# CHEBSB/PolarDecoding

Hardware: AMD Instinct MI355X
Metric: decoded frames/sec, N=1024 K=512 CA-SCL L=8 (higher is better)
Workload: dtype f64

## Files before the change

### polardecoding_amd/csrc/scl_fast2.h

```cpp
#pragma once
#include "fast2_lds.h"
#include "fast2_scratch.h"
#include "octet_bits.h"
#include "scl_fast.h"

namespace polar {

template <typename R>
struct Fast2Cfg {
    static constexpr int NLOG = 10, N = 1024, NW = 32, TOP = 9, HI = 8, L = 8;
    static constexpr int NA = 32;
    static constexpr int WAVES = 4;
    static constexpr int MIN_WAVES_PER_SIMD = sizeof(R) == 8 ? 3 : 4;
    static constexpr int NFA = HI - 3;
    static constexpr size_t sc_l8 = fast2_scratch::SC_L8;
    static constexpr size_t sc_l7 = fast2_scratch::SC_L7;
    static constexpr size_t sc_l6 = fast2_scratch::SC_L6;
    static constexpr size_t sc_tl = fast2_scratch::SC_TL;
    static constexpr size_t scratch_cw = fast2_scratch::SCRATCH_CW;
    static constexpr size_t scratch_elems = 2 * scratch_cw;
    static constexpr bool PAIRED = sizeof(R) == 8;
    static constexpr bool TOP_WORDS_ONCE = sizeof(R) == 8;
    static constexpr size_t off_lut = 0;
    static constexpr size_t off_frz = off_lut + ((Lut<R>::bytes + 15) / 16) * 16;
    static constexpr size_t off_msk = off_frz + 4 * NW;
    static constexpr size_t off_kth = off_msk + 4 * CRC_MASK_ROWS * NW;
    static constexpr size_t off_stair = off_kth + 256 * 8;
    static constexpr size_t shared_bytes = off_stair + ((Stair<R>::bytes + 15) / 16) * 16;
    static constexpr size_t off_bl = 0;
    static constexpr size_t off_cw = off_bl + 4 * fast2_lds::ROWS_WORDS;
    static constexpr size_t off_cd = off_cw + 4 * fast2_lds::ROWS_WORDS;
    static constexpr size_t off_ky = off_cd + sizeof(R) * 32;
    static constexpr size_t off_sg = off_ky + 128;
    static constexpr size_t per_wave = off_sg + sizeof(R) * 512;
    static constexpr size_t total = shared_bytes + WAVES * per_wave;
    static_assert(off_cw % 16 == 0 && off_cd % 16 == 0 && per_wave % 16 == 0 && shared_bytes % 16 == 0, "LDS regions are 16-byte aligned");
};
static_assert(3 * Fast2Cfg<double>::total <= 163840 && 4 * Fast2Cfg<float>::total <= 163840, "the pair kernel's LDS limits its occupancy");

template <int QP>
__device__ __forceinline__ double quadp(double x) { return quad_lanes<QP>(x); }
template <int QP>
__device__ __forceinline__ float quadp(float x) { return quad_lanes<QP>(x); }

template <bool FROM_Y>
struct Fast2Sigma { double sigma; };
template <>
struct Fast2Sigma<false> {};

template <typename R, typename IN, bool CRC_ON, bool FROM_Y>
struct Fast2Dec : Fast2Sigma<FROM_Y> {
    using C = Fast2Cfg<R>;
    static constexpr int N = C::N, NW = C::NW, TOP = C::TOP, HI = C::HI, L = 8, NFA = C::NFA;

    R A[C::NA];
    R a1;
    R bp_s, bp_d, bp_ts, bp_td;
    R PM;
    uint32_t ptr, bl0, fl;
    int logact;
    int p, c, pos, lane, gl;
    int own_addr, oth_addr;
    uint32_t pos0_mask;
    int cand_addr;
    Lut<R> lut;
    R *cand, *stg;
    uint32_t *blw, *curw, *keys;
    const unsigned char *kth;
    __amdgpu_buffer_rsrc_t rs_scr;
    __amdgpu_buffer_rsrc_t rs_in;
    unsigned cscr;
    unsigned csrc;
    static __device__ __forceinline__ __amdgpu_buffer_rsrc_t make_rsrc(const void *base, unsigned bytes)
    {
        return __builtin_amdgcn_make_buffer_rsrc(const_cast<void *>(base), 0, (int)bytes, 0x00020000);
    }
    typedef unsigned u2_t __attribute__((ext_vector_type(2)));
    static __device__ __forceinline__ double ld_buf(__amdgpu_buffer_rsrc_t r, unsigned eoff, double, int aux)
    {
        return aux ? __builtin_bit_cast(double, __builtin_amdgcn_raw_buffer_load_b64(r, eoff * 8u, 0, 16))
                   : __builtin_bit_cast(double, __builtin_amdgcn_raw_buffer_load_b64(r, eoff * 8u, 0, 0));
    }
    static __device__ __forceinline__ float ld_buf(__amdgpu_buffer_rsrc_t r, unsigned eoff, float, int aux)
    {
        return aux ? __builtin_bit_cast(float, __builtin_amdgcn_raw_buffer_load_b32(r, eoff * 4u, 0, 16))
                   : __builtin_bit_cast(float, __builtin_amdgcn_raw_buffer_load_b32(r, eoff * 4u, 0, 0));
    }
    static __device__ __forceinline__ void st_buf(__amdgpu_buffer_rsrc_t r, unsigned eoff, double v)
    {
        __builtin_amdgcn_raw_buffer_store_b64(__builtin_bit_cast(u2_t, v), r, eoff * 8u, 0, 0);
    }
    static __device__ __forceinline__ void st_buf(__amdgpu_buffer_rsrc_t r, unsigned eoff, float v)
    {
        __builtin_amdgcn_raw_buffer_store_b32(__builtin_bit_cast(unsigned, v), r, eoff * 4u, 0, 0);
    }
    typedef unsigned u4_t __attribute__((ext_vector_type(4)));
    struct R2 {
        R a, b;
    };
    static __device__ __forceinline__ R2 ld_buf2(__amdgpu_buffer_rsrc_t r, unsigned eoff, int aux)
    {
        static_assert(sizeof(R2) == 16, "paired accesses are for f64");
        return aux ? __builtin_bit_cast(R2, __builtin_amdgcn_raw_buffer_load_b128(r, eoff * 8u, 0, 16))
                   : __builtin_bit_cast(R2, __builtin_amdgcn_raw_buffer_load_b128(r, eoff * 8u, 0, 0));
    }
    static __device__ __forceinline__ void st_buf2(__amdgpu_buffer_rsrc_t r, unsigned eoff, R2 v)
    {
        static_assert(sizeof(R2) == 16, "paired accesses are for f64");
        __builtin_amdgcn_raw_buffer_store_b128(__builtin_bit_cast(u4_t, v), r, eoff * 8u, 0, 0);
    }
    struct SPtr {
        const Fast2Dec *d;
        unsigned off;
        struct Ref {
            const Fast2Dec *d;
            unsigned off;
            __device__ __forceinline__ void operator=(R v) const { st_buf(d->rs_scr, off, v); }
        };
        __device__ __forceinline__ SPtr operator+(int k) const { return SPtr{d, off + (unsigned)k}; }
        __device__ __forceinline__ Ref operator[](int k) const { return Ref{d, off + (unsigned)k}; }
    };
    static __device__ __forceinline__ R ld_sc(SPtr q) { return ld_buf(q.d->rs_scr, q.off, R(0), 1); }
    static __device__ __forceinline__ int sg(int e) { return C::PAIRED ? (int)fast2_scratch::sigma((unsigned)e) : e; }
    static __device__ __forceinline__ int sg2(int pos, int m) { return C::PAIRED ? (int)fast2_scratch::pair_at((unsigned)pos, (unsigned)m) : pos + 8 * m; }
    static __device__ __forceinline__ R2 ld_sc2(SPtr q)
    {
        if constexpr (C::PAIRED) return ld_buf2(q.d->rs_scr, q.off, 1);
        else return R2{ld_sc(q), ld_sc(q + sg(4))};
    }
    static __device__ __forceinline__ void st_sc2(SPtr q, R a, R b)
    {
        if constexpr (C::PAIRED) st_buf2(q.d->rs_scr, q.off, R2{a, b});
        else {
            q[0] = a;
            q[sg(4)] = b;
        }
    }

    static __device__ __forceinline__ int row(int slot) { return fast2_lds::row(slot); }
    __device__ __forceinline__ int pa(int t) const { return (ptr >> (3 * (t - 4))) & 7; }
    __device__ __forceinline__ void set_pa(int t, int v) { ptr = (ptr & ~(7u << (3 * (t - 4)))) | ((uint32_t)v << (3 * (t - 4))); }
    __device__ __forceinline__ int pb(int t) const { return (ptr >> (3 * (NFA + t - 5))) & 7; }
    __device__ __forceinline__ void set_pb(int t, int v) { ptr = (ptr & ~(7u << (3 * (NFA + t - 5)))) | ((uint32_t)v << (3 * (NFA + t - 5))); }
    __device__ __forceinline__ R chk(R a, R b) const { return chk_lut1<R>(a, b, lut); }
    __device__ __forceinline__ R chks(R a, R b) const { return chk_lut1<R>(a, b, lut); }
    __device__ __forceinline__ R chv(int e) const
    {
        double v = (double)ld_buf(rs_in, csrc + (unsigned)e, IN(0), 0);
        if constexpr (FROM_Y) v = llr_from_y(v, this->sigma);
        return (R)v;
    }
    static __device__ __forceinline__ unsigned fresh(unsigned off)
    {
        __asm__ volatile("" : "+v"(off));
        return off;
    }
    __device__ __forceinline__ SPtr l8(int slot) const { return SPtr{this, fresh(cscr + (unsigned)(C::sc_l8 + slot * 256))}; }
    __device__ __forceinline__ SPtr l7(int slot) const { return SPtr{this, fresh(cscr + (unsigned)(C::sc_l7 + slot * 128))}; }
    __device__ __forceinline__ SPtr tls() const { return SPtr{this, fresh(cscr + (unsigned)C::sc_tl)}; }

    template <int T>
    __device__ __forceinline__ void f_reg()
    {
        constexpr int RO = (1 << T) / 4;
#pragma unroll
        for (int r = 0; r < RO; ++r) A[RO + r] = chk(A[2 * RO + r], A[3 * RO + r]);
        if constexpr (T >= 4) set_pa(T, p);
    }
    template <int T>
    __device__ __forceinline__ void g_reg()
    {
        constexpr int RO = (1 << T) / 4;
        const int sl = pa(T + 1) * 8 + gl;
        uint32_t w;
        if constexpr (T == 5) w = blw[row(pb(5)) + 1] >> pos;
        else w = bl0 >> (16 + pos);
#pragma unroll
        for (int r = 0; r < RO; ++r) {
            const R x = __shfl(A[2 * RO + r], sl), y = __shfl(A[3 * RO + r], sl);
            A[RO + r] = g_bit<R>(x, y, w, 4 * r);
        }
        set_pa(T, p);
    }
    __device__ __forceinline__ void g3()
    {
        const int sl = pa(4) * 8 + gl;
        const uint32_t w = bl0 >> (8 + pos);
#pragma unroll
        for (int r = 0; r < 2; ++r) {
            const R x = __shfl(A[4 + r], sl), y = __shfl(A[6 + r], sl);
            A[2 + r] = g_bit<R>(x, y, w, 4 * r);
        }
    }

    __device__ __forceinline__ void push_l6(R v)
    {
#pragma unroll
        for (int r = 16; r < 31; ++r) A[r] = A[r + 1];
        A[31] = v;
    }
    __device__ __forceinline__ void load_l6() { set_pa(6, p); }
    __device__ __forceinline__ R top_src(bool right, int idx, int q) const
    {
        const int seg = idx >> 4, within = idx & 15;
        const int e = 16 * q + within + 64 * (seg & 3) + 256 * (seg >> 2);
        return right ? chv(e) : ld_sc(tls() + e);
    }
    __device__ __forceinline__ void from_top(bool right, bool gstep)
    {
        vm_drain();
        const uint32_t *bt = blw + row(pb(TOP)) + 16;
        const uint32_t *bh = blw + row(pb(HI)) + 8;
        const SPtr o8 = l8(p), o7 = l7(p);
        const int w32 = (int)fresh((unsigned)(p * 4 + pos));
        const int nld = right ? 8 : 4;
        R *pre = A + 4;
#pragma unroll
        for (int m = 0; m < 8; ++m) pre[m] = (m < nld) ? top_src(right, w32 + 32 * m, 0) : R(0);
        uint32_t wt[8] = {0, 0, 0, 0, 0, 0, 0, 0}, wh[4] = {0, 0, 0, 0};
        for (int q = 0; q < 4; ++q) {
            lds_fence();
#pragma unroll
            for (int m = 0; m < 8; ++m)
                if (m < nld) stg[w32 + 32 * m] = pre[m];
            if (C::TOP_WORDS_ONCE && (q & 1) == 0) {
                const int wq = q >> 1;
#pragma unroll
                for (int k = 0; k < 4; ++k) {
                    if (right) {
                        wt[k] = bt[2 * k + wq] >> pos;
                        wt[4 + k] = bt[8 + 2 * k + wq] >> pos;
                    }
                    if (gstep) wh[k] = bh[2 * k + wq] >> pos;
                }
            }
            lds_fence();
            if (q < 3) {
#pragma unroll
                for (int m = 0; m < 8; ++m) pre[m] = (m < nld) ? top_src(right, w32 + 32 * m, q + 1) : R(0);
            }
#pragma unroll 1
            for (int i = 0; i < 4; ++i) {
                const int rr = 4 * q + i;
                const int s0 = sg(pos + 4 * rr);
                const int sh = 4 * (rr & 7);
                const int wq = rr >> 3;
                const int wi = 4 * i + pos;
                R *v8 = A + 12;
#pragma unroll
                for (int k = 0; k < 4; ++k) {
                    R x, y;
                    if (right) {
                        const uint32_t w0 = C::TOP_WORDS_ONCE ? wt[k] : bt[2 * k + wq] >> pos;
                        const uint32_t w1 = C::TOP_WORDS_ONCE ? wt[4 + k] : bt[8 + 2 * k + wq] >> pos;
                        x = g_bit<R>(stg[(k + 0) * 16 + wi], stg[(k + 8) * 16 + wi], w0, sh);
                        y = g_bit<R>(stg[(k + 4) * 16 + wi], stg[(k + 12) * 16 + wi], w1, sh);
                    } else {
                        x = stg[(k + 0) * 16 + wi];
                        y = stg[(k + 4) * 16 + wi];
                    }
                    if (gstep) v8[k] = g_bit<R>(x, y, C::TOP_WORDS_ONCE ? wh[k] : bh[2 * k + wq] >> pos, sh);
                    else v8[k] = chk(x, y);
                    o8[s0 + 64 * k] = v8[k];
                }
                const R v70 = chk(v8[0], v8[2]), v71 = chk(v8[1], v8[3]);
                o7[s0] = v70;
                o7[s0 + 64] = v71;
                push_l6(chk(v70, v71));
            }
        }
        set_pa(8, p);
        set_pa(7, p);
        load_l6();
    }
    __device__ __forceinline__ void from_l8()
    {
        vm_drain();
        const SPtr s8 = l8(pa(8));
        const uint32_t *b7 = blw + row(pb(7)) + 4;
        const SPtr o7 = l7(p);
        constexpr int CP = sizeof(R) == 8 ? 2 : 4;
        static_assert(CP % 2 == 0 && 4 * CP <= 16, "a chunk is whole pairs of passes and fits the dead registers");
        for (int q = 0; q < 16 / CP; ++q) {
            R *in = A;
#pragma unroll
            for (int j = 0; j < CP / 2; ++j) {
                const int m = CP / 2 * q + j;
#pragma unroll
                for (int k = 0; k < 4; ++k) {
                    const R2 v = ld_sc2(s8 + sg2(pos, m) + 64 * k);
                    in[8 * j + k] = v.a;
                    in[8 * j + 4 + k] = v.b;
                }
            }
#pragma unroll
            for (int j = 0; j < CP / 2; ++j) {
                const int m = CP / 2 * q + j;
                R v70[2], v71[2];
#pragma unroll
                for (int h = 0; h < 2; ++h) {
                    const int i = 2 * j + h;
                    const int rr = CP * q + i;
                    const int sh = 4 * (rr & 7);
                    const int wq = rr >> 3;
                    v70[h] = g_bit<R>(in[4 * i], in[4 * i + 2], b7[wq] >> pos, sh);
                    v71[h] = g_bit<R>(in[4 * i + 1], in[4 * i + 3], b7[2 + wq] >> pos, sh);
                }
                st_sc2(o7 + sg2(pos, m), v70[0], v70[1]);
                st_sc2(o7 + sg2(pos, m) + 64, v71[0], v71[1]);
                push_l6(chk(v70[0], v71[0]));
                push_l6(chk(v70[1], v71[1]));
            }
        }
        set_pa(7, p);
        load_l6();
    }
    __device__ __forceinline__ void from_l7()
    {
        vm_drain();
        const SPtr s7 = l7(pa(7));
        const uint32_t *b6 = blw + row(pb(6)) + 2;
        const uint32_t w0 = b6[0] >> pos, w1 = b6[1] >> pos;
#pragma unroll
        for (int m = 0; m < 8; ++m) {
            const R2 x = ld_sc2(s7 + sg2(pos, m)), y = ld_sc2(s7 + sg2(pos, m) + 64);
            const int r = 2 * m;
            A[16 + r] = g_bit<R>(x.a, y.a, r < 8 ? w0 : w1, 4 * (r & 7));
            A[17 + r] = g_bit<R>(x.b, y.b, r < 8 ? w0 : w1, 4 * ((r + 1) & 7));
        }
        set_pa(6, p);
    }

    __device__ __forceinline__ void octet_head(int o)
    {
        const int d = (o == 0) ? 10 : 3 + __builtin_ctz((unsigned)o);
        if (d >= 8) from_top(o >= N / 16, d == 8);
        else if (d == 7) from_l8();
        else if (d == 6) from_l7();
        else if (d == 5) g_reg<5>();
        else if (d == 4) g_reg<4>();
        else g3();
        if (d > 5) f_reg<5>();
        if (d > 4) f_reg<4>();
        if (d > 3) f_reg<3>();
    }
    __device__ __forceinline__ void octet_head_reg(int o)
    {
        const int d = 3 + __builtin_ctz((unsigned)o);
        if (d == 5) g_reg<5>();
        else if (d == 4) g_reg<4>();
        else g3();
        if (d > 4) f_reg<4>();
        if (d > 3) f_reg<3>();
    }

    template <int K>
    __device__ __forceinline__ void set_bit_k(int o, uint32_t bit)
    {
        if constexpr (K < 7) {
            bl0 |= bit << K;
        } else {
            const uint32_t c3 = octet_bits::level3((bl0 & 0x7Fu) | (bit << 7));
            bl0 &= ~0xFFu;
            set_bit7(o, c3);
        }
    }
    __device__ __forceinline__ void set_bit7(int o, uint32_t c3)
    {
        if ((o & 1) == 0) {
            bl0 = (bl0 & ~0xFF00u) | (c3 << 8);
            return;
        }
        const uint32_t c4 = (((bl0 >> 8) & 0xFFu) ^ c3) | (c3 << 8);
        if ((o & 2) == 0) {
            bl0 = (bl0 & 0xFFFFu) | (c4 << 16);
            return;
        }
        set_bit_lds(8 * o + 7, ((bl0 >> 16) ^ c4) | (c4 << 16));
    }
    __device__ __forceinline__ void set_bit_lds(int j, uint32_t cur)
    {
        const int own = (int)fresh((unsigned)row(p));
        lds_fence();
        if (pos == 0) curw[own] = cur;
        lds_fence();
        int t = 5;
        while (t < 10 && ((j >> t) & 1)) {
            const int nw = 1 << (t - 5);
            const int sb = pb(t);
            for (int w = pos; w < nw; w += 4) {
                const uint32_t cc = curw[own + w];
                const uint32_t l = blw[row(sb) + nw + w];
                curw[own + w] = l ^ cc;
                curw[own + w + nw] = cc;
            }
            lds_fence();
            ++t;
        }
        if (t < 10) {
            const int nw = 1 << (t - 5);
            for (int w = pos; w < nw; w += 4) blw[own + nw + w] = curw[own + w];
            set_pb(t, p);
            lds_fence();
        }
    }

    __device__ __forceinline__ uint32_t survivors(R c0, R c1)
    {
        lds_fence();
        if (pos == 0) {
            keys[2 * p] = metric_key(c0);
            keys[2 * p + 1] = metric_key(c1);
        }
        lds_fence();
        const unsigned char *kb = reinterpret_cast<const unsigned char *>(keys) - 64 * c;
        const uint32_t own = *reinterpret_cast<const uint32_t *>(kb + own_addr);
        const uint32_t oth = *reinterpret_cast<const uint32_t *>(kb + oth_addr);
        const uint32_t own1 = own + 1u;
        uint32_t acc = (oth - own1) >> 31;
        acc = __builtin_amdgcn_alignbit(acc, (uint32_t)dpp_i<0x121>((int)oth) - own1, 31);
        acc = __builtin_amdgcn_alignbit(acc, (uint32_t)dpp_i<0x122>((int)oth) - own1, 31);
        acc = __builtin_amdgcn_alignbit(acc, (uint32_t)dpp_i<0x123>((int)oth) - own1, 31);
        acc = __builtin_amdgcn_alignbit(acc, (uint32_t)dpp_i<0x124>((int)oth) - own1, 31);
        acc = __builtin_amdgcn_alignbit(acc, (uint32_t)dpp_i<0x125>((int)oth) - own1, 31);
        acc = __builtin_amdgcn_alignbit(acc, (uint32_t)dpp_i<0x126>((int)oth) - own1, 31);
        acc = __builtin_amdgcn_alignbit(acc, (uint32_t)dpp_i<0x127>((int)oth) - own1, 31);
        uint32_t cnt = __popc(acc);
        {
            auto r = __builtin_amdgcn_permlane16_swap(cnt, cnt, false, false);
            cnt = r[0] + r[1];
        }
        uint64_t b = __ballot(cnt <= (uint32_t)L);
        uint32_t m_a = (uint32_t)b & 0xFFFFu, m_b = (uint32_t)(b >> 32) & 0xFFFFu;
        if (sizeof(R) == 8 && (__popc(m_a) != L || __popc(m_b) != L)) {
            if (__popc(c ? m_b : m_a) != L) fl |= 0x4u;
            lds_fence();
            if (pos == 0) {
                cand[p] = c0;
                cand[8 + p] = c1;
            }
            lds_fence();
            const R *cb = reinterpret_cast<const R *>(reinterpret_cast<const unsigned char *>(cand) - (int)sizeof(R) * 16 * c);
            const R *mycand = reinterpret_cast<const R *>(reinterpret_cast<const unsigned char *>(cb) + cand_addr);
            const R mine = mycand[lane & 15];
            int n = 0;
#pragma unroll
            for (int m = 0; m < 16; ++m) n += (mycand[m] <= mine) ? 1 : 0;
            b = __ballot(n <= L);
            m_a = (uint32_t)b & 0xFFFFu;
            m_b = (uint32_t)(b >> 32) & 0xFFFFu;
        }
        return c ? m_b : m_a;
    }

    __device__ __forceinline__ bool trivial_prune(R cb, R cw) const
    {
        uint32_t mx = metric_key(cb) & pos0_mask;
        mx = max(mx, (uint32_t)dpp_i<0x128>((int)mx));
        {
            auto a = __builtin_amdgcn_permlane16_swap(mx, mx, false, false);
            mx = max(a[0], a[1]);
        }
        {
            auto a = __builtin_amdgcn_permlane32_swap(mx, mx, false, false);
            mx = max(a[0], a[1]);
        }
        return __ballot(mx >= (metric_key(cw) | ~pos0_mask)) == 0ull;
    }
    static __device__ __forceinline__ uint32_t sign_bit(double x) { return (uint32_t)__double2hiint(x) >> 31; }
    static __device__ __forceinline__ uint32_t sign_bit(float x) { return (uint32_t)__float_as_int(x) >> 31; }

    template <int K, bool FULL>
    __device__ __forceinline__ void decide(int o, bool frozen, R lam) { decide_t<K, FULL>(o, frozen, lam, lut.tabv(lam)); }
    template <int K, bool FULL>
    __device__ __forceinline__ void decide_t(int o, bool frozen, R lam, R tt)
    {
        if (frozen) {
            PM += tt + negmax(lam);
            set_bit_k<K>(o, 0u);
            return;
        }
        uint32_t bit;
        R pm;
        if (!FULL && logact < 3) {
            const R ph0 = tt + negmax(lam), ph1 = tt + posmax(lam);
            bit = (p >> logact) & 1;
            pm = PM + (bit ? ph1 : ph0);
            ++logact;
        } else {
            const uint32_t lneg = sign_bit(lam);
            const R cb = PM + tt, cw = PM + (tt + absr(lam));
            bit = (uint32_t)dpp_i<0x00>((int)lneg);
            pm = cb;
            if (!trivial_prune(cb, cw)) ranked<K>(lneg, cb, cw, bit, pm);
        }
        PM = pm;
        set_bit_k<K>(o, bit);
    }
    template <int K>
    __device__ __forceinline__ void ranked(uint32_t lneg, R cb, R cw, uint32_t &bit, R &pm)
    {
        const R c0 = lneg ? cw : cb, c1 = lneg ? cb : cw;
        const uint32_t mask = survivors(c0, c1);
        const uint32_t m0 = mask & 0xFFu, m1 = mask >> 8;
        const uint32_t m_both = m0 & m1, m_dead = ~(m0 | m1) & 0xFFu;
        if (__popc(mask) < L) fl |= 0x1u;
        const bool s0 = (m0 >> p) & 1, s1 = (m1 >> p) & 1;
        bit = (!s0 && s1) ? 1u : 0u;
        pm = bit ? c1 : c0;
        if (__ballot(m_dead != 0u) == 0ull) return;
        const bool dead = !s0 && !s1;
        const int myrank = __popc(m_dead & ((1u << p) - 1u));
        const bool refilled = dead && (myrank < __popc(m_both));
        const int src = (int)kth[m_both * 8 + myrank];
        const int sg = refilled ? src : p;
        const int sl = sg * 8 + gl;
        const R c1s = __shfl(c1, sl);
        ptr = __shfl(ptr, sl);
        bl0 = __shfl(bl0, sl);
        if constexpr ((K & 4) == 0) { A[2] = __shfl(A[2], sl); A[3] = __shfl(A[3], sl); }
        if constexpr ((K & 2) == 0) { A[1] = __shfl(A[1], sl); a1 = __shfl(a1, sl); }
        if constexpr ((K & 1) == 0) { bp_d = __shfl(bp_d, sl); bp_td = __shfl(bp_td, sl); }
        bit = refilled ? 1u : bit;
        pm = refilled ? c1s : pm;
    }

    __device__ __forceinline__ void frozen_prefix(int P, int nphi, bool regs, R &xl, R &yl)
    {
        const int w32 = p * 4 + pos, j0 = 8 * P;
        vm_drain();
        {
            const SPtr tl = tls();
            const SPtr o8 = l8(0) + sg(w32), o7 = l7(0) + sg(w32);
            R v8[8];
#pragma unroll
            for (int k = 0; k < 8; ++k) {
                const int e = w32 + 32 * k;
                v8[k] = chk(ld_sc(tl + e), ld_sc(tl + e + 256));
                o8[32 * k] = v8[k];
            }
            lds_fence();
#pragma unroll
            for (int k = 0; k < 4; ++k) {
                const R v7 = chk(v8[k], v8[k + 4]);
                o7[32 * k] = v7;
                stg[w32 + 32 * k] = v7;
            }
            set_pa(8, 0);
            set_pa(7, 0);
        }
        lds_fence();
#pragma unroll
        for (int t = 6; t >= 0; --t) {
            const int h = 1 << t;
            int idx[2];
            R x[2], y[2];
#pragma unroll
            for (int i = 0; i < 2; ++i) {
                const int b = w32 + 32 * i;
                idx[i] = ((b >> t) << (t + 1)) | (b & (h - 1));
                x[i] = stg[idx[i]];
                y[i] = stg[idx[i] + h];
            }
            if (t == 0) {
                xl = stg[126];
                yl = stg[127];
            }
            lds_fence();
#pragma unroll
            for (int i = 0; i < 2; ++i) {
                stg[idx[i]] = chk(x[i], y[i]);
                stg[idx[i] + h] = y[i] + x[i];
            }
            lds_fence();
            if (t >= 4 && regs) {
                const R *node = stg + ((j0 >> t) << t) + pos;
#pragma unroll
                for (int r = 0; r < h / 4; ++r) A[h / 4 + r] = node[4 * r];
            }
        }
#pragma unroll
        for (int k = 0; k < 4; ++k) {
            const R lam = stg[w32 + 32 * k];
            stg[128 + w32 + 32 * k] = lut.tabv(lam) + negmax(lam);
        }
        lds_fence();
        R pm = PM;
#pragma unroll 8
        for (int j = 0; j < nphi; ++j) pm += stg[128 + j];
        PM = pm;
        lds_fence();
    }

    __device__ __forceinline__ uint32_t fill_tail(uint32_t f2, R lam0, R xl, R yl)
    {
        uint32_t b0 = 0, b1 = 0;
        if (!(f2 & 1u)) {
            b0 = (p >> logact) & 1;
            ++logact;
        }
        PM += lut.tabv(lam0) + (b0 ? posmax(lam0) : negmax(lam0));
        const R lam1 = b0 ? -(xl - yl) : yl + xl;
        if (!(f2 & 2u)) {
            b1 = (p >> logact) & 1;
            ++logact;
        }
        PM += lut.tabv(lam1) + (b1 ? posmax(lam1) : negmax(lam1));
        return (b0 ? 0x55555555u : 0u) ^ (b1 ? 0xFFFFFFFFu : 0u);
    }
    __device__ __forceinline__ void fill_phase(int E, const uint32_t *frz, R xl, R yl)
    {
        const int w32 = (int)fresh((unsigned)(p * 4 + pos));
        const int qb = (p & 1) * 64;
        const uint32_t wv0 = fill_tail(frz[3] >> 30, stg[126], xl, yl);
        uint32_t wv1 = 0;
        lds_fence();
        blw[row(p) + 4 + pos] = wv0;
        lds_fence();
#pragma unroll 1
        for (int S = 128; S < E; S += 64) {
            vm_drain();
            const uint32_t wsel = S == 128 ? wv0 : wv1;
            uint32_t wq[2];
            wq[0] = (uint32_t)__shfl((int)wsel, gl) >> w32;
            wq[1] = (uint32_t)__shfl((int)wsel, 8 + gl) >> w32;
            if (S == 128) {
                const SPtr s8 = l8(0) + sg(w32);
                R v8[8];
#pragma unroll
                for (int k = 0; k < 8; ++k) v8[k] = ld_sc(s8 + 32 * k);
#pragma unroll
                for (int q = 0; q < 2; ++q) {
                    const SPtr o7 = l7(q) + sg(w32);
                    R v7[4];
#pragma unroll
                    for (int k = 0; k < 4; ++k) {
                        v7[k] = g_bit<R>(v8[k], v8[k + 4], wq[q], 0);
                        o7[32 * k] = v7[k];
                    }
                    stg[64 * q + w32] = chk(v7[0], v7[2]);
                    stg[64 * q + w32 + 32] = chk(v7[1], v7[3]);
                }
                set_pa(7, p & 1);
            } else {
#pragma unroll
                for (int q = 0; q < 2; ++q) {
                    const SPtr s7 = l7(q) + sg(w32);
#pragma unroll
                    for (int i = 0; i < 2; ++i)
                        stg[64 * q + w32 + 32 * i] = g_bit<R>(ld_sc(s7 + 32 * i), ld_sc(s7 + 32 * i + 64), wq[q], 0);
                }
            }
            lds_fence();
#pragma unroll
            for (int t = 5; t >= 0; --t) {
                const int h = 1 << t;
                int idx[2];
                R x[2], y[2];
#pragma unroll
                for (int i = 0; i < 2; ++i) {
                    const int b = w32 + 32 * i;
                    idx[i] = ((b >> t) << (t + 1)) | (b & (h - 1));
                    x[i] = stg[idx[i]];
                    y[i] = stg[idx[i] + h];
                }
                if (t == 0) {
                    xl = stg[qb + 62];
                    yl = stg[qb + 63];
                }
                lds_fence();
#pragma unroll
                for (int i = 0; i < 2; ++i) {
                    stg[idx[i]] = chk(x[i], y[i]);
                    stg[idx[i] + h] = y[i] + x[i];
                }
                lds_fence();
            }
#pragma unroll
            for (int k = 0; k < 4; ++k) {
                const R lam = stg[w32 + 32 * k];
                stg[128 + w32 + 32 * k] = lut.tabv(lam) + negmax(lam);
            }
            lds_fence();
            R pm = PM;
#pragma unroll 2
            for (int j = 0; j < 62; ++j) pm += stg[128 + qb + j];
            PM = pm;
            const uint32_t wv = fill_tail(frz[(S + 62) >> 5] >> 30, stg[qb + 62], xl, yl);
            lds_fence();
            if (S == 128) {
                wv1 = wv;
                if (pos < 2) blw[row(p) + 2 + pos] = wv;
            } else {
                const uint32_t b = pos < 2 ? wv1 ^ wv : wv;
                blw[row(p) + 8 + pos] = wv0 ^ b;
                blw[row(p) + 12 + pos] = b;
            }
            lds_fence();
        }
    }

    template <bool FULL>
    __device__ __forceinline__ void octet_frozen_prefix(int o, bool last_frozen)
    {
        R xf = chks(A[2], A[3]), xg = A[3] + A[2];
        R yf = quadp<0x4E>(xf), yg = quadp<0x4E>(xg);
        {
            const R ff = chks(xf, yf), gf = xf + yf, fg = chks(xg, yg), gg = xg + yg;
            xf = (pos & 2) ? gf : ff;
            xg = (pos & 2) ? gg : fg;
        }
        yf = quadp<0xB1>(xf); yg = quadp<0xB1>(xg);
        R lf, lg;
        {
            const R ff = chks(xf, yf), gf = xf + yf, fg = chks(xg, yg), gg = xg + yg;
            lf = (pos & 1) ? gf : ff;
            lg = (pos & 1) ? gg : fg;
        }
        const R pf = lut.tabv(lf) + negmax(lf), pg = lut.tabv(lg) + negmax(lg);
        PM += pf;
        PM += quadp<0x55>(pf);
        PM += quadp<0xAA>(pf);
        PM += quadp<0xFF>(pf);
        PM += pg;
        PM += quadp<0x55>(pg);
        PM += quadp<0xAA>(pg);
        if (last_frozen) {
            PM += quadp<0xFF>(pg);
            set_bit7(o, 0u);
        } else {
            decide<7, FULL>(o, false, quadp<0xFF>(lg));
        }
    }

    struct ChkBp { R v, s, d, ts, td; };
    static __device__ __forceinline__ R g_sel(R sum, R dif, uint32_t w, int sh)
    {
        const uint32_t m = (uint32_t)__builtin_amdgcn_sbfe((int)w, sh, 1);
        return Lut<R>::sel_mask(m, -dif, sum);
    }
    static __device__ __forceinline__ double flip_sign(double y, uint32_t m) { return __hiloint2double(__double2hiint(y) ^ (int)m, __double2loint(y)); }
    static __device__ __forceinline__ float flip_sign(float y, uint32_t m) { return __int_as_float(__float_as_int(y) ^ (int)m); }
    template <int QP>
    __device__ __forceinline__ ChkBp chk_narrow(R x) const
    {
        static_assert(QP == 0xB1 || QP == 0x4E, "partner in lane ^ 1 or lane ^ 2");
        const uint32_t up = QP == 0xB1 ? (uint32_t)pos << 31 : ((uint32_t)pos << 30) & 0x80000000u;
        const R y = flip_sign(quadp<QP>(x), up);
        ChkBp r;
        r.s = x + y;
        r.d = x - y;
        r.ts = lut.tabv(r.s);
        r.td = quadp<QP>(r.ts);
        r.v = xor_sign(minabs(x, y), x, y) + (r.ts - r.td);
        return r;
    }
    template <int K, bool FULL>
    __device__ __forceinline__ void leaf_pair(int o, uint32_t fm, R x1)
    {
        const ChkBp q = chk_narrow<0xB1>(x1);
        bp_d = q.d;
        bp_td = q.td;
        decide<K, FULL>(o, (fm >> K) & 1, q.v);
        const uint32_t m1 = (uint32_t)__builtin_amdgcn_sbfe((int)bl0, K, 1);
        decide_t<K + 1, FULL>(o, (fm >> (K + 1)) & 1, Lut<R>::sel_mask(m1, -bp_d, q.s), Lut<R>::sel_mask(m1, bp_td, q.ts));
    }
    template <bool FULL>
    __device__ __forceinline__ void octet(int o, uint32_t fm)
    {
        {
            const R s2 = A[2] + A[3], d2 = A[2] - A[3];
            const R v2 = xor_sign(minabs(A[2], A[3]), A[2], A[3]) + (lut.tabv(s2) - lut.tabv(d2));
            A[2] = s2;
            A[3] = d2;
            const ChkBp q1 = chk_narrow<0x4E>(v2);
            A[1] = q1.s;
            a1 = q1.d;
            leaf_pair<0, FULL>(o, fm, q1.v);
        }
        leaf_pair<2, FULL>(o, fm, g_sel(A[1], a1, octet_bits::level1_lo(bl0), pos));
        {
            const R v2 = g_sel(A[2], A[3], octet_bits::level2(bl0), pos);
            const ChkBp q1 = chk_narrow<0x4E>(v2);
            A[1] = q1.s;
            a1 = q1.d;
            leaf_pair<4, FULL>(o, fm, q1.v);
        }
        leaf_pair<6, FULL>(o, fm, g_sel(A[1], a1, octet_bits::level1_hi(bl0), pos));
    }
};

template <typename D, bool FULL>
__device__ __forceinline__ int octet_group(D &s, const uint32_t *frz, uint32_t &fword, int o)
{
    s.octet_head(o);
    for (;;) {
        if ((o & 3) == 0) fword = frz[o >> 2];
        const uint32_t fm = (fword >> (8 * (o & 3))) & 0xFFu;
        if ((fm & 0x7Fu) != 0x7Fu) s.template octet<FULL>(o, fm);
        else s.template octet_frozen_prefix<FULL>(o, fm == 0xFFu);
        ++o;
        if ((o & 7) == 0) break;
        s.octet_head_reg(o);
    }
    return o;
}

template <typename R, typename IN, bool CRC_ON, bool FROM_Y>
__device__ __forceinline__ void scl_fast2_body(const SclParams &P)
{
    using D = Fast2Dec<R, IN, CRC_ON, FROM_Y>;
    using C = Fast2Cfg<R>;
    constexpr int N = C::N, NW = C::NW, L = 8;
    extern __shared__ __attribute__((aligned(16))) unsigned char smem[];
    const int wave = __builtin_amdgcn_readfirstlane(threadIdx.x >> 6);
    unsigned char *base = smem + C::shared_bytes + (size_t)wave * C::per_wave;
    uint32_t *frz = reinterpret_cast<uint32_t *>(smem + C::off_frz);
    uint32_t *msk = reinterpret_cast<uint32_t *>(smem + C::off_msk);
    unsigned char *kth = smem + C::off_kth;

    Lut<R>::build(smem + C::off_lut, threadIdx.x, blockDim.x);
    for (int i = threadIdx.x; i < NW; i += blockDim.x) frz[i] = P.frozen[i];
    if (CRC_ON)
        for (int i = threadIdx.x; i < CRC_MASK_ROWS * NW; i += blockDim.x)
            msk[i] = P.crc_mask[(i & ~(NW - 1)) + ((i >> 3) & 3) + 4 * (i & 7)];
    for (int i = threadIdx.x; i < 256 * 8; i += blockDim.x) {
        int m = i >> 3, k = i & 7, idx = 0, seen = 0;
        for (int b = 0; b < 8; ++b)
            if ((m >> b) & 1) {
                if (seen == k) idx = b;
                ++seen;
            }
        kth[i] = (unsigned char)idx;
    }
    __syncthreads();

    D s;
    s.lane = threadIdx.x & 63;
    s.p = s.lane >> 3;
    s.c = (s.lane >> 2) & 1;
    s.pos = s.lane & 3;
    s.pos0_mask = s.pos == 0 ? 0xFFFFFFFFu : 0u;
    s.gl = s.lane & 7;
    s.lut.bind(smem + C::off_lut);
    s.kth = kth;
    s.blw = reinterpret_cast<uint32_t *>(base + C::off_bl) + fast2_lds::cw_base(1) * s.c;
    s.curw = reinterpret_cast<uint32_t *>(base + C::off_cw) + fast2_lds::cw_base(1) * s.c;
    s.cand = reinterpret_cast<R *>(base + C::off_cd) + s.c * 16;
    s.keys = reinterpret_cast<uint32_t *>(base + C::off_ky) + s.c * 16;
    s.stg = reinterpret_cast<R *>(base + C::off_sg) + s.c * 256;
    if constexpr (FROM_Y) s.sigma = P.sigma;
    {
        const int i = s.lane & 15, row = s.lane >> 4, cwr = row >> 1, h = row & 1;
        const int jj = (i + 8 * h) & 15;
        s.own_addr = 64 * cwr + 4 * (2 * (i & 7) + (i >> 3));
        s.oth_addr = 64 * cwr + 4 * (2 * (jj & 7) + (jj >> 3));
        s.cand_addr = (int)sizeof(R) * 16 * cwr;
    }
    const int lane = s.lane, p = s.p, c = s.c, pos = s.pos;
    const int wave_global = blockIdx.x * C::WAVES + wave;
    const int waves_total = gridDim.x * C::WAVES;
    R *scr_wave = reinterpret_cast<R *>(P.scratch) + (size_t)wave_global * C::scratch_elems;
    s.rs_scr = D::make_rsrc(scr_wave, (unsigned)(C::scratch_elems * sizeof(R)));
    s.cscr = (unsigned)c * (unsigned)C::scratch_cw;

    int lead = 0;
    while (lead < 15 && ((frz[lead >> 2] >> (8 * (lead & 3))) & 0xFFu) == 0xFFu) ++lead;
    lead = __builtin_amdgcn_readfirstlane(lead);
    const int E = P.fill_end;

    for (int pair = wave_global; 2 * pair < P.B;) {
        const int frame_raw = 2 * pair + c;
        const bool live = frame_raw < P.B;
        const int frame = live ? frame_raw : P.B - 1;
        s.rs_in = D::make_rsrc(reinterpret_cast<const IN *>(P.in) + (size_t)(2 * pair) * N, (unsigned)(2 * N * sizeof(IN)));
        s.csrc = (unsigned)(frame - 2 * pair) * (unsigned)N;
        {
            const auto t = s.tls();
            const int w = p * 4 + pos;
#pragma unroll 2
            for (int e = w; e < N / 2; e += 32) t[e] = s.chk(s.chv(e), s.chv(e + N / 2));
        }
#pragma unroll
        for (int j = 0; j < NW / 4; ++j) s.blw[D::row(p) + pos + 4 * j] = 0;
        lds_fence();

        s.PM = R(0);
        s.ptr = 0;
        for (int t = 4; t <= 8; ++t) s.set_pa(t, p);
        for (int t = 5; t <= 9; ++t) s.set_pb(t, p);
        s.bl0 = 0;
        s.a1 = R(0);
#pragma unroll
        for (int r = 0; r < C::NA; ++r) s.A[r] = R(0);
        s.fl = 0;
        s.logact = 0;
        uint32_t fword = 0;

        int o_first = 0;
        if (E > 0 || lead > 0) {
            R xl, yl;
            s.frozen_prefix(E > 0 ? 15 : lead, E > 0 ? 126 : 8 * lead, E == 0, xl, yl);
            o_first = lead;
            if (E > 0) {
                s.fill_phase(E, frz, xl, yl);
                o_first = E >> 3;
            }
            fword = frz[o_first >> 2];
        }
        int o = o_first;
#pragma unroll 1
        while (o < N / 8 && s.logact < 3) o = octet_group<D, false>(s, frz, fword, o);
        while (o < N / 8) o = octet_group<D, true>(s, frz, fword, o);

        bool pass = false;
        if constexpr (CRC_ON) {
            lds_fence();
            uint32_t x[8];
#pragma unroll
            for (int j = 0; j < 8; ++j) x[j] = s.curw[D::row(p) + pos + 4 * j];
            typedef uint32_t u4_t __attribute__((ext_vector_type(4)));
            const u4_t *mk = reinterpret_cast<const u4_t *>(msk + 8 * pos);
            const int rows = (P.crc_r + 3) & ~3;
            uint32_t rem = 0;
#pragma unroll 1
            for (int i = 0; i < rows; i += 4) {
#pragma unroll
                for (int k = 0; k < 4; ++k) {
                    const u4_t a = mk[(i + k) * (NW / 4)], b = mk[(i + k) * (NW / 4) + 1];
                    const uint32_t acc = (x[0] & a.x) ^ (x[1] & a.y) ^ (x[2] & a.z) ^ (x[3] & a.w) ^ (x[4] & b.x) ^
                                         (x[5] & b.y) ^ (x[6] & b.z) ^ (x[7] & b.w);
                    rem |= (uint32_t)(__popc(acc) & 1) << (i + k);
                }
            }
            rem ^= (uint32_t)dpp_i<0xB1>((int)rem);
            rem ^= (uint32_t)dpp_i<0x4E>((int)rem);
            pass = rem == 0u;
        }
        const uint64_t bp_ = __ballot(pass && pos == 0);
        const uint64_t cwmask = 0x0101010101010101ull << (4 * c);
        const bool any = (bp_ & cwmask) != 0ull;
        int best = -1;
        R best_pm = R(0);
        for (int q = 0; q < L; ++q) {
            const R pq = __shfl(s.PM, q * 8 + 4 * c);
            const int okq = __shfl((int)(any ? pass : true), q * 8 + 4 * c);
            if (okq && (best < 0 || pq < best_pm)) {
                best = q;
                best_pm = pq;
            }
        }
        uint32_t fl = s.fl;
        if (any) fl |= 0x2u;
        lds_fence();
        {
            const int w = p * 4 + pos;
            uint32_t x = s.curw[D::row(best) + w];
            x = polar_word_transform(x);
#pragma unroll
            for (int hw = 1; hw < NW; hw <<= 1) {
                const int wo = w ^ hw;
                const uint32_t ov = __shfl(x, (wo >> 2) * 8 + 4 * c + (wo & 3));
                if (!(w & hw)) x ^= ov;
            }
            if (live) P.out_bits[(size_t)frame * NW + w] = x;
        }
        if (live && p == 0 && pos == 0) {
            if (P.pm) P.pm[frame] = (double)best_pm;
            if (P.flags) P.flags[frame] = fl;
        }
        lds_fence();
        pair = next_job_wave(P.queue, pair, waves_total, (P.B + 1) >> 1);
    }
}

template <typename R, typename IN, bool CRC_ON>
__global__ __launch_bounds__(256, (Fast2Cfg<R>::MIN_WAVES_PER_SIMD)) void k_scl_fast2(SclParams P)
{
    scl_fast2_body<R, IN, CRC_ON, false>(P);
}
template <typename R, typename IN, bool CRC_ON>
__global__ __launch_bounds__(256, (Fast2Cfg<R>::MIN_WAVES_PER_SIMD)) void k_scl_fast2_y(SclParams P)
{
    scl_fast2_body<R, IN, CRC_ON, true>(P);
}

}
```

Baseline: 16.04 million.

## Precompute all four g/f candidates in staging for right non-gstep top descent

For the right-branch, non-g-step case of the top-level descent, the staging stores now hold all four combinations of the pairwise sums and differences, each already passed through the check-node function. Each path lane then reads the one candidate picked by a 2-bit selector taken from its partial-sum bits, instead of doing two g-steps and a check-node per output. A new header defines a skewed, XOR-swizzled index layout and checks at compile time that it is a bijection and free of LDS bank conflicts. The aim is to move arithmetic out of the per-path inner loop into shared staging work and to remove data-dependent selects. The cost is more LDS stores per staging lane and an extra fresh() lane computation per iteration.

```diff
diff --git a/polardecoding_amd/csrc/fast2_top.h b/polardecoding_amd/csrc/fast2_top.h
--- /dev/null
+++ b/polardecoding_amd/csrc/fast2_top.h
@@ -0,0 +1,91 @@
+#pragma once
+
+namespace polar {
+namespace fast2_top {
+
+constexpr int CHUNK = 256;
+constexpr int SEG = 16;
+constexpr int BANK_ELEMS = 32;
+
+constexpr int skew(int c) { return 16 * c; }
+constexpr int SEL8 = 64 + 4;
+constexpr int cand8(int c, int k, int wi, int sel) { return (wi + ((16 * k) ^ skew(c))) ^ (SEL8 * sel); }
+constexpr int staging_lane(int c, int w32) { return w32 ^ skew(c); }
+constexpr int put8(int ws, int j, int sel) { return (32 * j + ws) ^ (SEL8 * sel); }
+constexpr unsigned sel_pairs(unsigned w0, unsigned w1) { return (w0 & 0x11111111u) | ((w1 & 0x11111111u) << 1); }
+constexpr int slot(int c, int idx) { return CHUNK * c + idx; }
+
+constexpr bool octet64_bijection()
+{
+    for (int c = 0; c < 2; ++c) {
+        bool seen[CHUNK] = {};
+        for (int k = 0; k < 4; ++k)
+            for (int wi = 0; wi < SEG; ++wi)
+                for (int sel = 0; sel < 4; ++sel) {
+                    const int s = cand8(c, k, wi, sel);
+                    if (s < 0 || s >= CHUNK || seen[s]) return false;
+                    seen[s] = true;
+                }
+    }
+    return true;
+}
+constexpr bool writer_meets_reader()
+{
+    for (int c = 0; c < 2; ++c)
+        for (int w32 = 0; w32 < 32; ++w32)
+            for (int sel = 0; sel < 4; ++sel) {
+                for (int j = 0; j < 2; ++j)
+                    if (put8(staging_lane(c, w32), j, sel) != cand8(c, (w32 >> 4) + 2 * j, w32 & 15, sel)) return false;
+            }
+    return true;
+}
+constexpr bool halves_apart()
+{
+    for (int c = 0; c < 2; ++c)
+        for (int wi = 0; wi < SEG; ++wi)
+            for (int sel = 0; sel < 4; ++sel) {
+                for (int k = 0; k < 4; ++k)
+                    if (cand8(c, k, wi, sel) < 0 || cand8(c, k, wi, sel) >= CHUNK) return false;
+            }
+    return slot(0, CHUNK - 1) < slot(1, 0);
+}
+constexpr bool reads_conflict_free()
+{
+    for (int i = 0; i < 4; ++i) {
+        for (int k = 0; k < 4; ++k) {
+            unsigned seen = 0;
+            for (int c = 0; c < 2; ++c)
+                for (int pos = 0; pos < 4; ++pos)
+                    for (int sel = 0; sel < 4; ++sel) {
+                        const unsigned b = 1u << (slot(c, cand8(c, k, 4 * i + pos, sel)) % BANK_ELEMS);
+                        if (seen & b) return false;
+                        seen |= b;
+                    }
+        }
+    }
+    return true;
+}
+constexpr bool writes_conflict_free()
+{
+    for (int g = 0; g < 2; ++g)
+        for (int sel = 0; sel < 4; ++sel) {
+            for (int j = 0; j < 2; ++j) {
+                unsigned seen = 0;
+                for (int c = 0; c < 2; ++c)
+                    for (int w32 = 16 * g; w32 < 16 * g + 16; ++w32) {
+                        const unsigned b = 1u << (slot(c, put8(staging_lane(c, w32), j, sel)) % BANK_ELEMS);
+                        if (seen & b) return false;
+                        seen |= b;
+                    }
+            }
+        }
+    return true;
+}
+static_assert(octet64_bijection(), "octet 64: the candidate index is not a bijection onto the chunk's 256 slots");
+static_assert(writer_meets_reader(), "a staging lane's slots are not the ones the path lanes read");
+static_assert(halves_apart(), "a candidate leaves its codeword's half of the staging buffer");
+static_assert(reads_conflict_free(), "two slots of one read share a bank");
+static_assert(writes_conflict_free(), "two slots of one store share a bank");
+
+}
+}
diff --git a/polardecoding_amd/csrc/scl_fast2.h b/polardecoding_amd/csrc/scl_fast2.h
--- a/polardecoding_amd/csrc/scl_fast2.h
+++ b/polardecoding_amd/csrc/scl_fast2.h
@@ -1,6 +1,7 @@
 #pragma once
 #include "fast2_lds.h"
 #include "fast2_scratch.h"
+#include "fast2_top.h"
 #include "octet_bits.h"
 #include "scl_fast.h"
 
@@ -209,29 +210,49 @@
     __device__ __forceinline__ void from_top(bool right, bool gstep)
     {
         vm_drain();
+        const bool c64 = right && !gstep;
         const uint32_t *bt = blw + row(pb(TOP)) + 16;
         const uint32_t *bh = blw + row(pb(HI)) + 8;
         const SPtr o8 = l8(p), o7 = l7(p);
-        const int w32 = (int)fresh((unsigned)(p * 4 + pos));
+        const int w32_ = (int)fresh((unsigned)(p * 4 + pos));
+        const int cw_ = (int)fresh((unsigned)gl >> 2);
         const int nld = right ? 8 : 4;
         R *pre = A + 4;
 #pragma unroll
-        for (int m = 0; m < 8; ++m) pre[m] = (m < nld) ? top_src(right, w32 + 32 * m, 0) : R(0);
+        for (int m = 0; m < 8; ++m) pre[m] = (m < nld) ? top_src(right, w32_ + 32 * m, 0) : R(0);
+        const auto pairs64 = [&](int k, int wq) { return fast2_top::sel_pairs(bt[2 * k + wq] >> pos, bt[8 + 2 * k + wq] >> pos); };
         uint32_t wt[8] = {0, 0, 0, 0, 0, 0, 0, 0}, wh[4] = {0, 0, 0, 0};
         for (int q = 0; q < 4; ++q) {
-            lds_fence();
-#pragma unroll
-            for (int m = 0; m < 8; ++m)
-                if (m < nld) stg[w32 + 32 * m] = pre[m];
+            const int w32 = sizeof(R) == 8 ? (int)fresh((unsigned)(p * 4 + pos)) : w32_;
+            lds_fence();
+            const int ws = (int)fresh((unsigned)fast2_top::staging_lane(cw_, w32));
+            if (c64) {
+#pragma unroll
+                for (int j = 0; j < 2; ++j) {
+                    const R s1 = pre[4 + j] + pre[j], d1 = pre[4 + j] - pre[j];
+                    const R s2 = pre[6 + j] + pre[2 + j], d2 = pre[6 + j] - pre[2 + j];
+                    stg[fast2_top::put8(ws, j, 0)] = chk(s1, s2);
+                    stg[fast2_top::put8(ws, j, 1)] = chk(d1, s2);
+                    stg[fast2_top::put8(ws, j, 2)] = chk(s1, d2);
+                    stg[fast2_top::put8(ws, j, 3)] = chk(d1, d2);
+                }
+            } else {
+#pragma unroll
+                for (int m = 0; m < 8; ++m)
+                    if (m < nld) stg[w32 + 32 * m] = pre[m];
+            }
             if (C::TOP_WORDS_ONCE && (q & 1) == 0) {
                 const int wq = q >> 1;
 #pragma unroll
                 for (int k = 0; k < 4; ++k) {
-                    if (right) {
-                        wt[k] = bt[2 * k + wq] >> pos;
-                        wt[4 + k] = bt[8 + 2 * k + wq] >> pos;
+                    if (c64) wt[k] = pairs64(k, wq);
+                    else {
+                        if (right) {
+                            wt[k] = bt[2 * k + wq] >> pos;
+                            wt[4 + k] = bt[8 + 2 * k + wq] >> pos;
+                        }
+                        if (gstep) wh[k] = bh[2 * k + wq] >> pos;
                     }
-                    if (gstep) wh[k] = bh[2 * k + wq] >> pos;
                 }
             }
             lds_fence();
@@ -247,22 +268,32 @@
                 const int wq = rr >> 3;
                 const int wi = 4 * i + pos;
                 R *v8 = A + 12;
-#pragma unroll
-                for (int k = 0; k < 4; ++k) {
-                    R x, y;
-                    if (right) {
-                        const uint32_t w0 = C::TOP_WORDS_ONCE ? wt[k] : bt[2 * k + wq] >> pos;
-                        const uint32_t w1 = C::TOP_WORDS_ONCE ? wt[4 + k] : bt[8 + 2 * k + wq] >> pos;
-                        x = g_bit<R>(stg[(k + 0) * 16 + wi], stg[(k + 8) * 16 + wi], w0, sh);
-                        y = g_bit<R>(stg[(k + 4) * 16 + wi], stg[(k + 12) * 16 + wi], w1, sh);
-                    } else {
-                        x = stg[(k + 0) * 16 + wi];
-                        y = stg[(k + 4) * 16 + wi];
+                const int cw = (int)fresh((unsigned)gl >> 2);
+                if (c64) {
+#pragma unroll
+                    for (int k = 0; k < 4; ++k) {
+                        const uint32_t w = C::TOP_WORDS_ONCE ? wt[k] : pairs64(k, wq);
+                        v8[k] = stg[fast2_top::cand8(cw, k, wi, (int)((w >> sh) & 3u))];
                     }
-                    if (gstep) v8[k] = g_bit<R>(x, y, C::TOP_WORDS_ONCE ? wh[k] : bh[2 * k + wq] >> pos, sh);
-                    else v8[k] = chk(x, y);
-                    o8[s0 + 64 * k] = v8[k];
+                } else {
+#pragma unroll
+                    for (int k = 0; k < 4; ++k) {
+                        R x, y;
+                        if (right) {
+                            const uint32_t w0 = C::TOP_WORDS_ONCE ? wt[k] : bt[2 * k + wq] >> pos;
+                            const uint32_t w1 = C::TOP_WORDS_ONCE ? wt[4 + k] : bt[8 + 2 * k + wq] >> pos;
+                            x = g_bit<R>(stg[(k + 0) * 16 + wi], stg[(k + 8) * 16 + wi], w0, sh);
+                            y = g_bit<R>(stg[(k + 4) * 16 + wi], stg[(k + 12) * 16 + wi], w1, sh);
+                        } else {
+                            x = stg[(k + 0) * 16 + wi];
+                            y = stg[(k + 4) * 16 + wi];
+                        }
+                        if (gstep) v8[k] = g_bit<R>(x, y, C::TOP_WORDS_ONCE ? wh[k] : bh[2 * k + wq] >> pos, sh);
+                        else v8[k] = chk(x, y);
+                    }
                 }
+#pragma unroll
+                for (int k = 0; k < 4; ++k) o8[s0 + 64 * k] = v8[k];
                 const R v70 = chk(v8[0], v8[2]), v71 = chk(v8[1], v8[3]);
                 o7[s0] = v70;
                 o7[s0 + 64] = v71;
```

Measured after the change: 16.07 million (median of 2 runs). About the same (+0.2%).
